# jgsimard/big-dreamer

Measured on AMD Instinct MI355X. Metric: latent transitions/sec (RSSM + imagination) at batch=50 chunk=50 H=15, higher is better.
Workload: dtype f32

## Files before the change

### big_dreamer_amd/_cabi.py

```python
from __future__ import annotations

import ctypes as C
import os

import torch

_HERE = os.path.dirname(os.path.abspath(__file__))
LIB_PATH = os.environ.get("BD_LIB") or os.path.join(_HERE, "libbigdreamer_hip.so")

if not os.path.exists(LIB_PATH):
    raise ImportError(
        f"{LIB_PATH} is missing: the MI355X HIP extension has not been built "
        "(run `python -c 'import __graft_entry__ as g; g.build()'`). There is no CPU fallback.")

lib = C.CDLL(LIB_PATH)

BD_MAX_LAYERS = 6
ACT_NONE, ACT_ELU, ACT_ELU_GRAD = 0, 1, 2
ACT_RELU, ACT_RELU_GRAD, ACT_TANH, ACT_TANH_GRAD = 3, 4, 5, 6
CNN_ACTS = {"ELU": (ACT_ELU, ACT_ELU_GRAD), "ReLU": (ACT_RELU, ACT_RELU_GRAD), "Tanh": (ACT_TANH, ACT_TANH_GRAD)}
GRAD_ACTS = (ACT_ELU_GRAD, ACT_RELU_GRAD, ACT_TANH_GRAD)
P = C.c_void_p
F32 = C.c_float
I32 = C.c_int
# ... 265 lines not shown
    "bd_actor_entropy_rng": (I32, [C.c_ulonglong, C.c_ulonglong, C.c_uint, P, P, I32, I32, I32, I32, P]),
    "bd_gemm_nt": (I32, [P, I32, P, I32, P, I32, I32, I32, I32, I32, P]),
    "bd_categorical_head_forward": (I32, [P, P, I32, I32, I32, P, P, P]),
    "bd_categorical_head_backward": (I32, [P, P, I32, I32, I32, P, P]),
    "bd_kl_categorical_forward": (I32, [P, P, I32, I32, I32, F32, I32, P, I32, P, P]),
    "bd_kl_categorical_backward": (I32, [P, P, I32, I32, I32, F32, F32, F32, F32, P, I32, P, P, P]),
    "bd_plan_rollout": (I32, [C.POINTER(PlanArgs), P]),
    "bd_cem_refit": (I32, [P, I32, P, I32, I32, I32, I32, I32, P, P, P]),
    "bd_plan_rollout_cat": (I32, [C.POINTER(PlanCatArgs), P]),
    "bd_act_step_supported": (I32, [I32, I32, I32, I32, I32, I32]),
    "bd_act_step": (I32, [C.POINTER(ActArgs), P]),
    "bd_act_step_cat_supported": (I32, [I32] * 10),
    "bd_act_step_cat": (I32, [C.POINTER(ActCatArgs), P]),
    "bd_tanh_normal_mode": (I32, [P, P, P, C.c_ulonglong, C.c_ulonglong, C.c_uint, I32, I32, I32, P, P, P]),
    "bd_lambda_return_backward": (I32, [P, F32, I32, I32, F32, F32, P, P, P]),
    "bd_img_heads_supported": (I32, [I32, I32]),
    "bd_img_heads_fwd_bwd": (I32, [C.POINTER(ImgHeadsArgs), P]),
    "bd_actor_reinforce": (I32, [P, P, P, P, P, P, P, I32, I32, I32, F32, F32, F32, I32, P, P, I32, P, P]),
    "bd_actor_reinforce_cat": (I32, [P, P, P, P, P, P, I32, I32, I32, F32, F32, F32, I32, P, P, I32, P, P]),
    "bd_normal_nll": (I32, [P, I32, P, I32, I32, I32, F32, P, I32, P, I32, P, P]),
    "bd_bernoulli_nll": (I32, [P, P, C.c_size_t, F32, P, P, I32, P, P]),
    "bd_kl_forward": (I32, [P, P, P, P, I32, I32, F32, I32, P, I32, P, P]),
    "bd_kl_backward": (I32, [P, P, P, P, I32, I32, F32, F32, F32, F32, P, I32, P, P, P, P, P]),
    "bd_sum": (I32, [P, C.c_size_t, P, I32, P, P]),
    "bd_sumsq": (I32, [P, C.c_size_t, P, I32, P, P]),
    "bd_adam_step": (I32, [P, P, P, P, C.c_size_t, F32, F32, F32, F32, F32, I32, F32, P, I32, P]),
    "bd_polyak": (I32, [P, P, C.c_size_t, F32, P]),
    "bd_replay_gather": (I32, [P, P, I32, I32, P, P]),
    "bd_replay_gather_pixels": (I32, [P, P, I32, I32, I32, P, P, P]),
    "bd_replay_gather_pixels_rng": (I32, [P, P, I32, I32, I32, C.c_ulonglong, C.c_ulonglong, P, P]),
    "bd_replay_append": (I32, [C.POINTER(ReplayAppendArgs), P]),
    "bd_replay_sample_gather": (I32, [C.POINTER(ReplaySampleArgs), P]),
    "bd_reduce_ws_floats": (C.c_size_t, []),
    "bd_conv_gemm": (I32, [C.POINTER(ConvArgs), P]),
    "bd_conv_thin_forward": (I32, [P, I32, I32, I32, I32, I32, P, I32, P, I32, P, P, P]),
    "bd_conv_pack_class": (I32, [P, P, I32, I32, I32, I32, I32, I32, I32, P]),
    "bd_conv_pack_fused": (I32, [P, P, I32, I32, I32, P]),
    "bd_act_backward": (I32, [P, P, C.c_size_t, I32, P]),
    "bd_elu_backward": (I32, [P, P, C.c_size_t, P]),
    "bd_image_layout": (I32, [P, P, I32, I32, I32, I32, P]),
    "bd_eval_frame": (I32, [P, P, I32, U8P, I32, I32, P]),
    "bd_openl_video": (I32, [P, P, I32, I32, U8P, P]),
    "bd_openl_error": (I32, [P, P, I32, I32, I32, I32, P, P]),
    "bd_colsum_ws_floats": (C.c_size_t, [I32]),
    "bd_colsum": (I32, [P, C.c_size_t, I32, P, P, P]),
    "bd_fingerprint": (I32, [C.POINTER(FingerprintArgs), P, P]),
    "bd_diag_ws_floats": (C.c_size_t, []),
    "bd_moments": (I32, [C.POINTER(MomentsArgs), P, P, P]),
    "bd_latent_stats": (I32, [P, P, P, P, I32, I32, P, P, P, P]),
    "bd_latent_stats_categorical": (I32, [P, P, I32, I32, I32, P, P, P, P, P]),
    "bd_segment_sumsq": (I32, [P, I32, C.POINTER(C.c_size_t), P, P, P]),
    "bd_return_range": (I32, [P, I32, I32, I32, C.c_double, C.c_double, P, P, P]),
    "bd_return_seed": (I32, [P, F32, P, C.c_size_t, P, P, I32, P]),
    "bd_actor_reinforce_norm": (I32, [P, P, P, P, P, P, P, P, I32, I32, I32, F32, F32, F32, I32, P, P, I32, P, P]),
    "bd_actor_reinforce_cat_norm": (I32, [P, P, P, P, P, P, P, I32, I32, I32, F32, F32, F32, I32, P, P, I32, P, P]),
    "bd_twohot_decode": (I32, [P, I32, I32, I32, F32, P, P, P]),
    "bd_twohot_decode_backward": (I32, [P, I32, P, I32, I32, F32, P, I32, P]),
    "bd_twohot_nll": (I32, [P, I32, P, P, I32, I32, F32, F32, P, I32, P, P, P]),
}

for _name, (_res, _args) in _SIGS.items():
    _fn = getattr(lib, _name)
    _fn.restype = _res
    _fn.argtypes = _args

EXPORTED = tuple(_SIGS)
# ... 25 lines not shown
```

### big_dreamer_amd/csrc/cabi.hip

```cpp
#include "bd_device.h"
#include "bd_host.h"
#include "bd_rng.h"

namespace bd {
char* err_buf() {
    static thread_local char buf[512] = "";
    return buf;
}

constexpr int kPackThreads = 256, kPackWaves = kPackThreads / 64;
constexpr int kPackCopyX = 16;
constexpr int kPackProdX = 192;
constexpr int kPackE = 256;
struct alignas(16) PackLds {
    float a[16][kPackE + 1];
    float b[kPackE][16];
    float part[kPackWaves][16][17];
};
__device__ __forceinline__ void pack_product(const bd_pack_desc& d, int bx, int nx, PackLds& L) {
    const int Nb = (d.N + 15) >> 4, Kb = (d.K + 15) >> 4;
    const int tid = threadIdx.x, wave = tid >> 6, lane = tid & 63;
    const float* __restrict__ A = d.src;
    const float* __restrict__ B = d.src2;
    const bool vec = ((reinterpret_cast<uintptr_t>(A) | reinterpret_cast<uintptr_t>(B)) & 15) == 0 && (d.ld & 3) == 0 &&
// ... 113 lines not shown
    }
}
template <bool RNG>
__global__ __launch_bounds__(256) void gather_pixels_kernel(const unsigned char* __restrict__ src,
                                                            const int64_t* __restrict__ idx, int n_idx, int pixels,
                                                            float inv_q, float inv_b, const float* __restrict__ noise,
                                                            float* __restrict__ dst, Rng rng) {
    const int quads = pixels >> 2;
    const size_t total = (size_t)n_idx * quads;
    for (size_t e = (size_t)blockIdx.x * blockDim.x + threadIdx.x; e < total; e += (size_t)gridDim.x * blockDim.x) {
        const size_t r = e / quads, q = e - r * quads;
        const uchar4 u = reinterpret_cast<const uchar4*>(src + (size_t)idx[r] * pixels)[q];
        floatx4 nz;
        if constexpr (RNG) {
            const Philox4 p = philox4x32_10((uint32_t)e, (uint32_t)(e >> 32), rng.stream, rng.step, rng.k0, rng.k1);
#pragma unroll
            for (int j = 0; j < 4; ++j) nz[j] = (float)(p.x[j] >> 8) * (1.0f / 16777216.0f);
        } else {
            nz = reinterpret_cast<const floatx4*>(noise)[e];
        }
        floatx4 o;
        o[0] = floorf((float)u.x * inv_q) * inv_b - 0.5f + nz[0] * inv_b;
        o[1] = floorf((float)u.y * inv_q) * inv_b - 0.5f + nz[1] * inv_b;
        o[2] = floorf((float)u.z * inv_q) * inv_b - 0.5f + nz[2] * inv_b;
        o[3] = floorf((float)u.w * inv_q) * inv_b - 0.5f + nz[3] * inv_b;
        reinterpret_cast<floatx4*>(dst)[e] = o;
    }
}
}

extern "C" {

const char* bd_last_error(void) { return bd::err_buf(); }
int bd_version(void) { return 3; }

size_t bd_packed_floats(int N, int K) { return (size_t)bd::cdiv(N, 16) * bd::cdiv(K, 16) * 256; }

int bd_pack_weights(const bd_pack_desc* descs, int n, void* stream) {
    const int n_prod = n > 0 ? n / BD_PACK_PRODUCTS : 0;
    n = n > 0 ? n % BD_PACK_PRODUCTS : n;
    BD_REQUIRE(descs != nullptr && n > 0 && n_prod <= n, "bd_pack_weights: no descriptors");
    hipLaunchKernelGGL(bd::pack_kernel, dim3((n - n_prod) * bd::kPackCopyX + n_prod * bd::kPackProdX), dim3(bd::kPackThreads),
                       n_prod > 0 ? sizeof(bd::PackLds) : 0, (hipStream_t)stream, descs, n - n_prod);
    BD_CHECK_LAUNCH("bd_pack_weights");
    return 0;
}

int bd_replay_gather(const float* src, const int64_t* idx, int n_idx, int width, float* dst, void* stream) {
    BD_REQUIRE(src && idx && dst && n_idx > 0 && width > 0, "bd_replay_gather: bad arguments");
    const size_t total = (size_t)n_idx * width;
    const int blocks = (int)((total + 255) / 256 < 2048 ? (total + 255) / 256 : 2048);
    hipLaunchKernelGGL(bd::gather_rows_kernel, dim3(blocks), dim3(256), 0, (hipStream_t)stream, src, idx, n_idx, width, dst);
    BD_CHECK_LAUNCH("bd_replay_gather");
    return 0;
}

int bd_replay_gather_pixels(const unsigned char* src, const int64_t* idx, int n_idx, int pixels, int bit_depth,
                            const float* noise, float* dst, void* stream) {
    BD_REQUIRE(src && idx && noise && dst && n_idx > 0 && pixels > 0 && (pixels & 3) == 0 && bit_depth >= 1 && bit_depth <= 8,
               "bd_replay_gather_pixels: bad arguments");
    const size_t total = (size_t)n_idx * (pixels >> 2);
    const int blocks = (int)((total + 255) / 256 < 4096 ? (total + 255) / 256 : 4096);
    hipLaunchKernelGGL(bd::gather_pixels_kernel<false>, dim3(blocks), dim3(256), 0, (hipStream_t)stream, src, idx, n_idx, pixels,
                       1.0f / (float)(1 << (8 - bit_depth)), 1.0f / (float)(1 << bit_depth), noise, dst, bd::Rng{0, 0, 0, 0});
    BD_CHECK_LAUNCH("bd_replay_gather_pixels");
    return 0;
}
// ... 16 lines not shown
```

### big_dreamer_amd/csrc/reduce.hip

```cpp
#include "bd_device.h"
#include "bd_host.h"
#include "bd_discrete.h"
#include "bd_latent.h"

namespace bd {

constexpr int kRedBlocks = 1024;
constexpr float kHalfLog2Pi = 0.91893853320467274178f;

static inline int red_blocks(size_t n) {
    size_t b = (n + 255) / 256;
    return (int)(b < 1 ? 1 : (b > kRedBlocks ? kRedBlocks : b));
}

__global__ __launch_bounds__(256) void final_sum_kernel(const double* __restrict__ partials, int n,
                                                        float* __restrict__ scalars, int slot) {
    __shared__ double red[kWaves];
    double s = 0.0;
    for (int i = threadIdx.x; i < n; i += blockDim.x) s += partials[i];
    s = block_sum_d(s, red);
    if (threadIdx.x == 0) scalars[slot] = (float)s;
}

template <int MODE>
__global__ __launch_bounds__(256) void sum_kernel(const float* __restrict__ x, size_t n, double* __restrict__ partials) {
    __shared__ double red[kWaves];
    double s = 0.0;
    for (size_t i = (size_t)blockIdx.x * blockDim.x + threadIdx.x; i < n; i += (size_t)gridDim.x * blockDim.x) {
        const float v = x[i];
        s += MODE ? (double)v * v : (double)v;
    }
    s = block_sum_d(s, red);
    if (threadIdx.x == 0) partials[blockIdx.x] = s;
}

__global__ __launch_bounds__(256) void normal_nll_kernel(const float* __restrict__ pred, int ldp,
                                                         const float* __restrict__ target, int ldt, int rows, int D,
                                                         float grad_scale, float* __restrict__ dpred, int ldd,
                                                         double* __restrict__ partials) {
    __shared__ double red[kWaves];
    double s = 0.0;
    const size_t n = (size_t)rows * D;
    for (size_t i = (size_t)blockIdx.x * blockDim.x + threadIdx.x; i < n; i += (size_t)gridDim.x * blockDim.x) {
        const size_t r = i / D, c = i - r * D;
        const float d = pred[r * ldp + c] - target[r * ldt + c];
        s += (double)(0.5f * d * d + kHalfLog2Pi);
        if (dpred) dpred[r * ldd + c] = d * grad_scale;
    }
    s = block_sum_d(s, red);
    if (threadIdx.x == 0) partials[blockIdx.x] = s;
}

__global__ __launch_bounds__(256) void bernoulli_nll_kernel(const float* __restrict__ logits, const float* __restrict__ target,
                                                            size_t n, float grad_scale, float* __restrict__ dlogits,
                                                            double* __restrict__ partials) {
    __shared__ double red[kWaves];
    double s = 0.0;
    for (size_t i = (size_t)blockIdx.x * blockDim.x + threadIdx.x; i < n; i += (size_t)gridDim.x * blockDim.x) {
        const float x = logits[i], t = target[i];
        s += (double)(fmaxf(x, 0.f) - x * t + log1pf(expf(-fabsf(x))));
        if (dlogits) dlogits[i] = (1.f / (1.f + expf(-x)) - t) * grad_scale;
    }
    s = block_sum_d(s, red);
    if (threadIdx.x == 0) partials[blockIdx.x] = s;
}

__global__ __launch_bounds__(256) void kl_fwd_kernel(const float* __restrict__ qm, const float* __restrict__ qs,
                                                     const float* __restrict__ pm, const float* __restrict__ ps,
                                                     int rows, int S, float free_nats, int sum_form,
                                                     double* __restrict__ partials) {
    __shared__ double red[kWaves];
    double s = 0.0;
    if (!sum_form) {
        const size_t n = (size_t)rows * S;
        for (size_t i = (size_t)blockIdx.x * blockDim.x + threadIdx.x; i < n; i += (size_t)gridDim.x * blockDim.x)
            s += (double)kl_elem(qm[i], qs[i], pm[i], ps[i]);
    } else {
        for (size_t r = (size_t)blockIdx.x * blockDim.x + threadIdx.x; r < (size_t)rows;
             r += (size_t)gridDim.x * blockDim.x) {
            float rs = 0.f;
            for (int c = 0; c < S; ++c) {
                const size_t i = r * S + c;
                rs += kl_elem(qm[i], qs[i], pm[i], ps[i]);
            }
            s += (double)fmaxf(rs, free_nats);
        }
    }
    s = block_sum_d(s, red);
    if (threadIdx.x == 0) partials[blockIdx.x] = s;
}

__device__ __forceinline__ float max_grad(float x, float fn) { return x < fn ? 0.f : (x == fn ? 0.5f : 1.f); }

__global__ __launch_bounds__(256) void kl_bwd_kernel(const float* __restrict__ qm, const float* __restrict__ qs,
                                                     const float* __restrict__ pm, const float* __restrict__ ps,
                                                     int rows, int S, float free_nats, float kl_balance, float weight,
                                                     float inv_count, const float* __restrict__ scalars, int slot,
                                                     float* __restrict__ dqm, float* __restrict__ dqs,
                                                     float* __restrict__ dpm, float* __restrict__ dps) {
    const size_t n = (size_t)rows * S;
    const bool sum_form = kl_balance == -1.f;
    float fq, fp;
    if (!sum_form) {
        const float f = max_grad(scalars[slot] * inv_count, free_nats) * weight * inv_count;
        fp = kl_balance * f;
        fq = (1.f - kl_balance) * f;
    } else {
        fq = fp = weight / (float)rows;
    }
    for (size_t i = (size_t)blockIdx.x * blockDim.x + threadIdx.x; i < n; i += (size_t)gridDim.x * blockDim.x) {
        float gq = fq, gp = fp;
        if (sum_form) {
            const size_t r = i / S;
            float rs = 0.f;
            for (int c = 0; c < S; ++c) {
                const size_t j = r * S + c;
                rs += kl_elem(qm[j], qs[j], pm[j], ps[j]);
            }
            const float f = max_grad(rs, free_nats);
            gq *= f;
            gp *= f;
        }
// ... 45 lines not shown
        for (int t = Hm - 1; t >= 0; --t) {
            const float next = (t == Hm - 1) ? boot : value[(size_t)(t + 1) * N + n];
            const float inp = reward[(size_t)t * N + n] + disc * next * one_minus;
            last = inp + dl * last;
            ret[(size_t)t * N + n] = last;
        }
    }
}

__global__ __launch_bounds__(256) void lambda_bwd_kernel(const float* __restrict__ dret, float dconst, int Hm, int N,
                                                         float disc, float lam, float* __restrict__ dreward,
                                                         float* __restrict__ dvalue) {
    const float c = disc * lam, w = disc * (1.f - lam);
    for (int n = blockIdx.x * blockDim.x + threadIdx.x; n < N; n += gridDim.x * blockDim.x) {
        float G = 0.f;
        for (int t = 0; t < Hm; ++t) {
            G = (dret ? dret[(size_t)t * N + n] : dconst) + c * G;
            dreward[(size_t)t * N + n] = G;
            if (t == 0 && Hm > 1) dvalue[n] = 0.f;
            if (t < Hm - 1) {
                dvalue[(size_t)(t + 1) * N + n] = G * w;
            } else {
                const float prev = (Hm > 1) ? dvalue[(size_t)t * N + n] : 0.f;
                dvalue[(size_t)t * N + n] = prev + G * w + c * G;
            }
        }
    }
}

__global__ __launch_bounds__(256) void actor_reinforce_kernel(
    const float* __restrict__ eps, const float* __restrict__ us, const float* __restrict__ stats,
    const float* __restrict__ ret, const float* __restrict__ base0, const float* __restrict__ value,
    const float* __restrict__ weight, const float* __restrict__ ret_scale, int rows, int N, int A, float scale,
    float dentropy, int write, float* __restrict__ dout, double* __restrict__ partials) {
    __shared__ double red[kWaves];
    constexpr float kLn2 = 0.69314718055994531f;
    if (ret_scale) scale /= ret_scale[0];
    double s = 0.0;
    for (int i = blockIdx.x * blockDim.x + threadIdx.x; i < rows; i += gridDim.x * blockDim.x) {
        const float w = weight ? weight[i] : 1.f;
        const float adv = ret[i] - (i < N ? base0[i] : value[i - N]);
        const float c = scale * w * adv;
        const float dent = dentropy * w;
        const float* e = eps + (size_t)i * A;
        const float* uu = us + (size_t)i * 2 * A;
        const float* st = stats + (size_t)i * 4 * A;
        float* d = dout + (size_t)i * 2 * A;
        float l = 0.f;
        for (int j = 0; j < A; ++j) {
            const float ej = e[j], u = uu[j], sd = uu[A + j];
            const float th = st[j], sg = st[A + j];
            const float x = -2.f * u;
            const float sp = fmaxf(x, 0.f) + log1pf(expf(-fabsf(x)));
            l += -0.5f * ej * ej - logf(sd) - kHalfLog2Pi - 2.f * (kLn2 - u - sp);
            const float inv = 1.f / sd, dth = 1.f - th * th;
            float gm = c * (ej * inv) * dth;
            float gr = c * ((ej * ej - 1.f) * inv) * sg;
            if (write) {
                gm += (dent * st[2 * A + j]) * dth;
                gr += (dent * st[3 * A + j]) * sg;
            } else {
                gm += d[j];
                gr += d[A + j];
            }
            d[j] = gm;
            d[A + j] = gr;
        }
        s += (double)(w * l * adv);
    }
    s = block_sum_d(s, red);
    if (threadIdx.x == 0) partials[blockIdx.x] = s;
}

__global__ __launch_bounds__(256) void actor_reinforce_cat_kernel(
    const float* __restrict__ action, const float* __restrict__ stats, const float* __restrict__ ret,
    const float* __restrict__ base0, const float* __restrict__ value, const float* __restrict__ weight,
    const float* __restrict__ ret_scale, int rows, int N, int A, float scale, float dentropy, int write,
    float* __restrict__ dout, double* __restrict__ partials) {
    __shared__ double red[kWaves];
    const int lane = threadIdx.x & 63;
    if (ret_scale) scale /= ret_scale[0];
    const int nw = gridDim.x * (blockDim.x >> 6);
    const bool valid = lane < A;
    double s = 0.0;
    for (int i = blockIdx.x * (blockDim.x >> 6) + (threadIdx.x >> 6); i < rows; i += nw) {
        const float w = weight ? weight[i] : 1.f;
        const float adv = ret[i] - (i < N ? base0[i] : value[i - N]);
        const float c = scale * w * adv;
        const size_t j = (size_t)i * A + lane;
        const float norm = valid ? stats[j] : -INFINITY;
        const unsigned long long hot = __ballot(valid && action[j] > 0.5f);
        const int k = hot ? __builtin_ctzll(hot) : 0;
        const float p = disc_probs(norm, valid);
        const float l = __shfl(norm, k, 64);
        float g = c * ((lane == k ? 1.f : 0.f) - p);
        if (write) {
            const float H = disc_entropy(norm, p, valid);
            g += (dentropy * w) * (-p * (norm + H));
        } else if (valid) {
            g += dout[j];
        }
        if (valid) dout[j] = g;
        if (lane == 0) s += (double)(w * l * adv);
    }
    s = block_sum_d(s, red);
    if (threadIdx.x == 0) partials[blockIdx.x] = s;
}

__global__ __launch_bounds__(256) void adam_kernel(float* __restrict__ p, float* __restrict__ g, float* __restrict__ m,
                                                   float* __restrict__ v, size_t n, float beta1, float beta2, float eps,
                                                   float wd, float step_size, float inv_sqrt_bc2, float max_norm,
                                                   const float* __restrict__ scalars, int sqnorm_slot) {
    const float total_norm = sqrtf(scalars[sqnorm_slot]);
    const float q = max_norm / (total_norm + 1e-6f);
    const float coef = q > 1.f ? 1.f : q;
    for (size_t i = (size_t)blockIdx.x * blockDim.x + threadIdx.x; i < n; i += (size_t)gridDim.x * blockDim.x) {
        const float gc = g[i] * coef;
        g[i] = gc;
        const float pi = p[i];
        const float gw = gc + wd * pi;
        const float mi = m[i] + (1.f - beta1) * (gw - m[i]);
        const float vi = v[i] * beta2 + (1.f - beta2) * gw * gw;
        m[i] = mi;
        v[i] = vi;
        const float denom = sqrtf(vi) * inv_sqrt_bc2 + eps;
        p[i] = pi - step_size * (mi / denom);
    }
}

__global__ __launch_bounds__(256) void polyak_kernel(float* __restrict__ t, const float* __restrict__ s, size_t n, float w) {
    for (size_t i = (size_t)blockIdx.x * blockDim.x + threadIdx.x; i < n; i += (size_t)gridDim.x * blockDim.x)
        t[i] = s[i] * w + t[i] * (1.f - w);
}

__global__ __launch_bounds__(256) void cat_head_fwd_kernel(const float* __restrict__ logits, const float* __restrict__ q,
                                                           size_t groups, int C, float* __restrict__ state,
                                                           float* __restrict__ probs) {
    const int l = threadIdx.x & 31;
    for (size_t g = (size_t)blockIdx.x * 8 + (threadIdx.x >> 5); g < groups; g += (size_t)gridDim.x * 8) {
// ... 29 lines not shown
            if (ob > best || (ob == best && oa < arg)) { best = ob; arg = oa; }
        }
#pragma unroll
        for (int i = 0; i < kCatPer; ++i) {
            const int c = l + 32 * i;
            if (c < C) state[base + c] = (c == arg) ? 1.f : 0.f;
        }
    }
}

__global__ __launch_bounds__(256) void cat_head_bwd_kernel(const float* __restrict__ dstate, const float* __restrict__ probs,
                                                           size_t groups, int C, float* __restrict__ dlogits) {
    const int l = threadIdx.x & 31;
    for (size_t g = (size_t)blockIdx.x * 8 + (threadIdx.x >> 5); g < groups; g += (size_t)gridDim.x * 8) {
        const size_t base = g * C;
        float pr[kCatPer], gr[kCatPer], dot = 0.f;
#pragma unroll
        for (int i = 0; i < kCatPer; ++i) {
            const int c = l + 32 * i;
            pr[i] = c < C ? probs[base + c] : 0.f;
            gr[i] = c < C ? dstate[base + c] : 0.f;
            dot += pr[i] * gr[i];
        }
        dot = half_sum(dot);
#pragma unroll
        for (int i = 0; i < kCatPer; ++i) {
            const int c = l + 32 * i;
            if (c < C) dlogits[base + c] = pr[i] * (gr[i] - dot);
        }
    }
}

__global__ __launch_bounds__(256) void cat_kl_fwd_kernel(const float* __restrict__ ql, const float* __restrict__ pl, int rows,
                                                         int D, int C, float free_nats, int sum_form,
                                                         double* __restrict__ partials) {
    __shared__ double red[kWaves > 4 ? kWaves : 4];
    const int l = threadIdx.x & 31;
    const size_t units = sum_form ? (size_t)rows : (size_t)rows * D;
    const int per = sum_form ? D : 1;
    double acc = 0.0;
    for (size_t u = (size_t)blockIdx.x * 8 + (threadIdx.x >> 5); u < units; u += (size_t)gridDim.x * 8) {
        float rs = 0.f;
        for (int d = 0; d < per; ++d) {
            const size_t base = (u * per + d) * C;
            float lq[kCatPer], lp[kCatPer];
            group_log_softmax(ql + base, C, l, lq);
            group_log_softmax(pl + base, C, l, lp);
            rs += group_kl(lq, lp, C, l);
        }
        if (l == 0) acc += (double)(sum_form ? fmaxf(rs, free_nats) : rs);
    }
    acc = block_sum_d(acc, red);
    if (threadIdx.x == 0) partials[blockIdx.x] = acc;
}

__global__ __launch_bounds__(256) void cat_kl_bwd_kernel(const float* __restrict__ ql, const float* __restrict__ pl, int rows,
                                                         int D, int C, float free_nats, float kl_balance, float weight,
                                                         float inv_count, const float* __restrict__ scalars, int slot,
                                                         float* __restrict__ dql, float* __restrict__ dpl) {
    const int l = threadIdx.x & 31;
    const bool sum_form = kl_balance == -1.f;
    const size_t units = sum_form ? (size_t)rows : (size_t)rows * D;
    const int per = sum_form ? D : 1;
    float fq, fp;
    if (!sum_form) {
        const float f = max_grad(scalars[slot] * inv_count, free_nats) * weight * inv_count;
        fp = kl_balance * f;
        fq = (1.f - kl_balance) * f;
    } else {
        fq = fp = weight / (float)rows;
    }
    for (size_t u = (size_t)blockIdx.x * 8 + (threadIdx.x >> 5); u < units; u += (size_t)gridDim.x * 8) {
        float f = 1.f;
        if (sum_form) {
            float rs = 0.f;
            for (int d = 0; d < per; ++d) {
                const size_t base = (u * per + d) * C;
                float lq[kCatPer], lp[kCatPer];
                group_log_softmax(ql + base, C, l, lq);
                group_log_softmax(pl + base, C, l, lp);
                rs += group_kl(lq, lp, C, l);
            }
            f = max_grad(rs, free_nats);
        }
        for (int d = 0; d < per; ++d) {
            const size_t base = (u * per + d) * C;
            float lq[kCatPer], lp[kCatPer];
            group_log_softmax(ql + base, C, l, lq);
            group_log_softmax(pl + base, C, l, lp);
            const float kl = group_kl(lq, lp, C, l);
#pragma unroll
            for (int i = 0; i < kCatPer; ++i) {
                const int c = l + 32 * i;
                if (c < C) {
                    const float qv = expf(lq[i]), pv = expf(lp[i]);
                    dql[base + c] = f * fq * (qv == 0.f ? 0.f : qv * (lq[i] - lp[i] - kl));
                    dpl[base + c] = f * fp * (pv - qv);
                }
            }
        }
    }
}

static int finish(double* partials, int nb, float* scalars, int slot, hipStream_t s, const char* name) {
    hipLaunchKernelGGL(final_sum_kernel, dim3(1), dim3(256), 0, s, partials, nb, scalars, slot);
    BD_CHECK_LAUNCH(name);
    return 0;
}

}

extern "C" {
using namespace bd;

size_t bd_reduce_ws_floats(void) { return 2 * (size_t)kRedBlocks; }

int bd_sum(const float* x, size_t n, float* scalars, int slot, float* ws, void* stream) {
    BD_REQUIRE(x && scalars && ws && n > 0, "bd_sum: bad arguments");
    const int nb = red_blocks(n);
    hipLaunchKernelGGL(sum_kernel<0>, dim3(nb), dim3(256), 0, (hipStream_t)stream, x, n, (double*)ws);
    BD_CHECK_LAUNCH("bd_sum");
    return finish((double*)ws, nb, scalars, slot, (hipStream_t)stream, "bd_sum(final)");
}

int bd_actor_reinforce_norm(const float* eps_action, const float* act_us, const float* act_stats, const float* returns,
                            const float* base0, const float* value, const float* weight, const float* ret_scale, int Hm,
                            int N, int A, float rho, float grad_scale, float dentropy, int write, float* d_actor_out,
                            float* scalars, int slot, float* ws, void* stream) {
    BD_REQUIRE(eps_action && act_us && act_stats && returns && base0 && (value || Hm == 1) && d_actor_out && scalars && ws,
               "bd_actor_reinforce: missing pointers");
    BD_REQUIRE(Hm > 0 && N > 0 && A > 0 && (size_t)Hm * N <= (size_t)INT32_MAX / 4 && slot >= 0,
               "bd_actor_reinforce: bad dims (Hm=%d N=%d A=%d slot=%d)", Hm, N, A, slot);
    BD_REQUIRE(rho >= 0.f && rho <= 1.f, "bd_actor_reinforce: gradient mixing %g outside [0, 1]", (double)rho);
    BD_REQUIRE(((size_t)ret_scale & 3u) == 0, "bd_actor_reinforce: ret_scale is not 4-byte aligned");
    const int rows = Hm * N;
    const int nb = red_blocks((size_t)rows);
    hipLaunchKernelGGL(actor_reinforce_kernel, dim3(nb), dim3(256), 0, (hipStream_t)stream, eps_action, act_us, act_stats,
                       returns, base0, value, weight, ret_scale, rows, N, A, -(1.f - rho) * grad_scale, dentropy, write,
                       d_actor_out, (double*)ws);
    BD_CHECK_LAUNCH("bd_actor_reinforce");
    return finish((double*)ws, nb, scalars, slot, (hipStream_t)stream, "bd_actor_reinforce(final)");
}

int bd_actor_reinforce(const float* eps_action, const float* act_us, const float* act_stats, const float* returns,
                       const float* base0, const float* value, const float* weight, int Hm, int N, int A, float rho,
                       float grad_scale, float dentropy, int write, float* d_actor_out, float* scalars, int slot, float* ws,
                       void* stream) {
    return bd_actor_reinforce_norm(eps_action, act_us, act_stats, returns, base0, value, weight, nullptr, Hm, N, A, rho,
                                   grad_scale, dentropy, write, d_actor_out, scalars, slot, ws, stream);
}

int bd_actor_reinforce_cat_norm(const float* action, const float* act_stats, const float* returns, const float* base0,
                                const float* value, const float* weight, const float* ret_scale, int Hm, int N, int A,
                                float rho, float grad_scale, float dentropy, int write, float* d_actor_out, float* scalars,
                                int slot, float* ws, void* stream) {
    BD_REQUIRE(action && act_stats && returns && base0 && (value || Hm == 1) && d_actor_out && scalars && ws,
               "bd_actor_reinforce_cat: missing pointers");
    BD_REQUIRE(Hm > 0 && N > 0 && A > 0 && A <= 64 && (size_t)Hm * N <= (size_t)INT32_MAX / 4 && slot >= 0,
               "bd_actor_reinforce_cat: bad dims (Hm=%d N=%d A=%d slot=%d)", Hm, N, A, slot);
    BD_REQUIRE(rho >= 0.f && rho <= 1.f, "bd_actor_reinforce_cat: gradient mixing %g outside [0, 1]", (double)rho);
    BD_REQUIRE(((size_t)ret_scale & 3u) == 0, "bd_actor_reinforce_cat: ret_scale is not 4-byte aligned");
    const int rows = Hm * N;
    const int nb = red_blocks((size_t)rows);
    hipLaunchKernelGGL(actor_reinforce_cat_kernel, dim3(nb), dim3(256), 0, (hipStream_t)stream, action, act_stats, returns,
                       base0, value, weight, ret_scale, rows, N, A, -(1.f - rho) * grad_scale, dentropy, write, d_actor_out,
                       (double*)ws);
    BD_CHECK_LAUNCH("bd_actor_reinforce_cat");
    return finish((double*)ws, nb, scalars, slot, (hipStream_t)stream, "bd_actor_reinforce_cat(final)");
}

int bd_actor_reinforce_cat(const float* action, const float* act_stats, const float* returns, const float* base0,
                           const float* value, const float* weight, int Hm, int N, int A, float rho, float grad_scale,
                           float dentropy, int write, float* d_actor_out, float* scalars, int slot, float* ws,
                           void* stream) {
    return bd_actor_reinforce_cat_norm(action, act_stats, returns, base0, value, weight, nullptr, Hm, N, A, rho, grad_scale,
                                       dentropy, write, d_actor_out, scalars, slot, ws, stream);
}

int bd_sumsq(const float* x, size_t n, float* scalars, int slot, float* ws, void* stream) {
    BD_REQUIRE(x && scalars && ws && n > 0, "bd_sumsq: bad arguments");
    const int nb = red_blocks(n);
    hipLaunchKernelGGL(sum_kernel<1>, dim3(nb), dim3(256), 0, (hipStream_t)stream, x, n, (double*)ws);
    BD_CHECK_LAUNCH("bd_sumsq");
    return finish((double*)ws, nb, scalars, slot, (hipStream_t)stream, "bd_sumsq(final)");
}

int bd_normal_nll(const float* pred, int ldp, const float* target, int ldt, int rows, int D, float grad_scale,
                  float* dpred, int ldd, float* scalars, int slot, float* ws, void* stream) {
    BD_REQUIRE(pred && target && scalars && ws && rows > 0 && D > 0, "bd_normal_nll: bad arguments");
    BD_REQUIRE(ldp >= D && ldt >= D && (!dpred || ldd >= D), "bd_normal_nll: leading dimension too small");
    const int nb = red_blocks((size_t)rows * D);
    hipLaunchKernelGGL(normal_nll_kernel, dim3(nb), dim3(256), 0, (hipStream_t)stream, pred, ldp, target, ldt, rows, D,
                       grad_scale, dpred, ldd, (double*)ws);
    BD_CHECK_LAUNCH("bd_normal_nll");
    return finish((double*)ws, nb, scalars, slot, (hipStream_t)stream, "bd_normal_nll(final)");
}

int bd_bernoulli_nll(const float* logits, const float* target, size_t n, float grad_scale, float* dlogits, float* scalars,
                     int slot, float* ws, void* stream) {
    BD_REQUIRE(logits && target && scalars && ws && n > 0, "bd_bernoulli_nll: bad arguments");
    const int nb = red_blocks(n);
    hipLaunchKernelGGL(bernoulli_nll_kernel, dim3(nb), dim3(256), 0, (hipStream_t)stream, logits, target, n, grad_scale,
                       dlogits, (double*)ws);
    BD_CHECK_LAUNCH("bd_bernoulli_nll");
    return finish((double*)ws, nb, scalars, slot, (hipStream_t)stream, "bd_bernoulli_nll(final)");
}

int bd_kl_forward(const float* qm, const float* qs, const float* pm, const float* ps, int rows, int S, float free_nats,
                  int sum_form, float* scalars, int slot, float* ws, void* stream) {
    BD_REQUIRE(qm && qs && pm && ps && scalars && ws && rows > 0 && S > 0, "bd_kl_forward: bad arguments");
    const int nb = red_blocks(sum_form ? (size_t)rows : (size_t)rows * S);
    hipLaunchKernelGGL(kl_fwd_kernel, dim3(nb), dim3(256), 0, (hipStream_t)stream, qm, qs, pm, ps, rows, S, free_nats,
                       sum_form, (double*)ws);
    BD_CHECK_LAUNCH("bd_kl_forward");
    return finish((double*)ws, nb, scalars, slot, (hipStream_t)stream, "bd_kl_forward(final)");
}

int bd_kl_backward(const float* qm, const float* qs, const float* pm, const float* ps, int rows, int S, float free_nats,
                   float kl_balance, float weight, float inv_count, const float* scalars, int slot, float* dqm,
                   float* dqs, float* dpm, float* dps, void* stream) {
    BD_REQUIRE(qm && qs && pm && ps && scalars && dqm && dqs && dpm && dps && rows > 0 && S > 0,
               "bd_kl_backward: bad arguments");
    hipLaunchKernelGGL(kl_bwd_kernel, dim3(red_blocks((size_t)rows * S)), dim3(256), 0, (hipStream_t)stream, qm, qs, pm,
                       ps, rows, S, free_nats, kl_balance, weight, inv_count, scalars, slot, dqm, dqs, dpm, dps);
    BD_CHECK_LAUNCH("bd_kl_backward");
    return 0;
}

int bd_gauss_head_forward(const float* out, const float* eps, int M, int S, float min_std, float* mean, float* std,
                          float* state, void* stream) {
    BD_REQUIRE(out && M > 0 && S > 0 && (!state || eps), "bd_gauss_head_forward: bad arguments");
    hipLaunchKernelGGL(gauss_head_fwd_kernel, dim3(red_blocks((size_t)M * S)), dim3(256), 0, (hipStream_t)stream, out, eps,
                       M, S, min_std, mean, std, state);
    BD_CHECK_LAUNCH("bd_gauss_head_forward");
    return 0;
}

int bd_gauss_head_backward(const float* out, const float* eps, const float* dstate, const float* dmean,
                           const float* dstd, int M, int S, float* dout, void* stream) {
    BD_REQUIRE(out && dout && M > 0 && S > 0 && (!dstate || eps), "bd_gauss_head_backward: bad arguments");
    hipLaunchKernelGGL(gauss_head_bwd_kernel, dim3(red_blocks((size_t)M * S)), dim3(256), 0, (hipStream_t)stream, out, eps,
                       dstate, dmean, dstd, M, S, dout);
    BD_CHECK_LAUNCH("bd_gauss_head_backward");
    return 0;
}

int bd_lambda_return_forward(const float* reward, const float* value, int Hm, int N, float discount, float lambda_,
                             float* returns, void* stream) {
// ... 32 lines not shown

static inline int cat_blocks(size_t units) {
    size_t b = (units + 7) / 8;
    return (int)(b < 1 ? 1 : (b > (size_t)kRedBlocks ? (size_t)kRedBlocks : b));
}

int bd_categorical_head_forward(const float* logits, const float* q_noise, int rows, int D, int C, float* state,
                                float* probs, void* stream) {
    BD_REQUIRE(logits && q_noise && state && probs && rows > 0 && D > 0, "bd_categorical_head_forward: bad arguments");
    BD_REQUIRE(C > 0 && C <= 32 * kCatPer, "bd_categorical_head_forward: %d classes (max %d)", C, 32 * kCatPer);
    const size_t groups = (size_t)rows * D;
    hipLaunchKernelGGL(cat_head_fwd_kernel, dim3(cat_blocks(groups)), dim3(256), 0, (hipStream_t)stream, logits, q_noise,
                       groups, C, state, probs);
    BD_CHECK_LAUNCH("bd_categorical_head_forward");
    return 0;
}

int bd_categorical_head_backward(const float* dstate, const float* probs, int rows, int D, int C, float* dlogits,
                                 void* stream) {
    BD_REQUIRE(dstate && probs && dlogits && rows > 0 && D > 0, "bd_categorical_head_backward: bad arguments");
    BD_REQUIRE(C > 0 && C <= 32 * kCatPer, "bd_categorical_head_backward: %d classes (max %d)", C, 32 * kCatPer);
    const size_t groups = (size_t)rows * D;
    hipLaunchKernelGGL(cat_head_bwd_kernel, dim3(cat_blocks(groups)), dim3(256), 0, (hipStream_t)stream, dstate, probs,
                       groups, C, dlogits);
    BD_CHECK_LAUNCH("bd_categorical_head_backward");
    return 0;
}

int bd_kl_categorical_forward(const float* post_logits, const float* prior_logits, int rows, int D, int C, float free_nats,
                              int sum_form, float* scalars, int slot, float* ws, void* stream) {
    BD_REQUIRE(post_logits && prior_logits && scalars && ws && rows > 0 && D > 0, "bd_kl_categorical_forward: bad arguments");
    BD_REQUIRE(C > 0 && C <= 32 * kCatPer, "bd_kl_categorical_forward: %d classes (max %d)", C, 32 * kCatPer);
    const int nb = cat_blocks(sum_form ? (size_t)rows : (size_t)rows * D);
    hipLaunchKernelGGL(cat_kl_fwd_kernel, dim3(nb), dim3(256), 0, (hipStream_t)stream, post_logits, prior_logits, rows, D, C,
                       free_nats, sum_form, (double*)ws);
    BD_CHECK_LAUNCH("bd_kl_categorical_forward");
    return finish((double*)ws, nb, scalars, slot, (hipStream_t)stream, "bd_kl_categorical_forward(final)");
}

int bd_kl_categorical_backward(const float* post_logits, const float* prior_logits, int rows, int D, int C, float free_nats,
                               float kl_balance, float weight, float inv_count, const float* scalars, int slot,
                               float* dpost, float* dprior, void* stream) {
    BD_REQUIRE(post_logits && prior_logits && scalars && dpost && dprior && rows > 0 && D > 0,
               "bd_kl_categorical_backward: bad arguments");
    BD_REQUIRE(C > 0 && C <= 32 * kCatPer, "bd_kl_categorical_backward: %d classes (max %d)", C, 32 * kCatPer);
    const bool sum_form = kl_balance == -1.f;
    hipLaunchKernelGGL(cat_kl_bwd_kernel, dim3(cat_blocks(sum_form ? (size_t)rows : (size_t)rows * D)), dim3(256), 0,
                       (hipStream_t)stream, post_logits, prior_logits, rows, D, C, free_nats, kl_balance, weight, inv_count,
                       scalars, slot, dpost, dprior);
    BD_CHECK_LAUNCH("bd_kl_categorical_backward");
    return 0;
}

}
```

### include/bigdreamer_hip.h

```cpp
#ifndef BIGDREAMER_HIP_H
#define BIGDREAMER_HIP_H

#include <stddef.h>
#include <stdint.h>

#ifdef __cplusplus
extern "C" {
#endif

#define BD_MAX_LAYERS 6
#define BD_ACT_NONE 0
#define BD_ACT_ELU 1
#define BD_ACT_ELU_GRAD 2
#define BD_ACT_RELU 3
#define BD_ACT_RELU_GRAD 4
#define BD_ACT_TANH 5
#define BD_ACT_TANH_GRAD 6

const char* bd_last_error(void);
int bd_version(void);

#define BD_PACK_COPY 0
#define BD_PACK_PRODUCT 1
#define BD_PACK_PRODUCT_VEC 2
// ... 541 lines not shown
    float* dst_reward;
    float* dst_nonterminal;
} bd_replay_append_args;
int bd_replay_append(const bd_replay_append_args* a, void* stream);

typedef struct {
    const void* obs;
    const float* act;
    const float* reward;
    const float* nonterminal;
    int obs_width;
    int A;
    int size;
    int lanes;
    int lane_size;
    int idx;
    int full;
    int n;
    int L;
    int bit_depth;
    unsigned long long seed;
    unsigned long long step;
    unsigned long long pix_seed;
    unsigned long long pix_step;
    float* dst_obs;
    float* dst_act;
    float* dst_reward;
    float* dst_nonterminal;
    int64_t* idx_out;
} bd_replay_sample_args;
int bd_replay_sample_gather(const bd_replay_sample_args* a, void* stream);

size_t bd_reduce_ws_floats(void);

#define BD_FP_MAX_BUFFERS 16
typedef struct {
    int n_buf;
    struct {
        const float* p;
        size_t n;
    } buf[BD_FP_MAX_BUFFERS];
} bd_fingerprint_args;
int bd_fingerprint(const bd_fingerprint_args* a, unsigned long long* out, void* stream);

size_t bd_diag_ws_floats(void);

#define BD_MOMENTS_MAX_BUFFERS 16
#define BD_MOMENTS_WORDS 6
typedef struct {
    int n_buf;
    struct {
        const float* p;
        const float* q;
        size_t n;
    } buf[BD_MOMENTS_MAX_BUFFERS];
} bd_moments_args;
int bd_moments(const bd_moments_args* a, double* out, float* ws, void* stream);

#define BD_LATENT_WORDS 15
int bd_latent_stats(const float* qm, const float* qs, const float* pm, const float* ps, int rows, int S, double* out,
                    double* colsum, float* ws, void* stream);

#define BD_LATENT_CAT_WORDS 5
int bd_latent_stats_categorical(const float* post_logits, const float* prior_logits, int rows, int D, int C, double* out,
                                double* colsum, unsigned* used, float* ws, void* stream);

// ... 19 lines not shown
```

Baseline: 13.92 million.

## Fuse reduction finalisation into one launch with a last-block ticket

Reduction kernels (sum, sumsq, NLL, KL, actor reinforce) now finish the reduction themselves. Each block writes its partial, fences, and takes an atomic ticket; the last block to arrive sums all partials and writes the scalar. This removes the separate single-block final_sum launch whenever the grid has at most 320 blocks, cutting per-loss launch overhead and a serial dependency. In exchange it adds atomics and fences and relies on the self-wrapping ticket counter starting at zero; a mode switch and a reset entry point allow falling back to the two-launch path.

```diff
diff --git a/big_dreamer_amd/_cabi.py b/big_dreamer_amd/_cabi.py
--- a/big_dreamer_amd/_cabi.py
+++ b/big_dreamer_amd/_cabi.py
@@ -321,6 +321,8 @@
     "bd_replay_append": (I32, [C.POINTER(ReplayAppendArgs), P]),
     "bd_replay_sample_gather": (I32, [C.POINTER(ReplaySampleArgs), P]),
     "bd_reduce_ws_floats": (C.c_size_t, []),
+    "bd_reduce_set_two_launch": (I32, [I32]),
+    "bd_reduce_reset": (I32, [C.c_void_p, C.c_void_p]),
     "bd_conv_gemm": (I32, [C.POINTER(ConvArgs), P]),
     "bd_conv_thin_forward": (I32, [P, I32, I32, I32, I32, I32, P, I32, P, I32, P, P, P]),
     "bd_conv_pack_class": (I32, [P, P, I32, I32, I32, I32, I32, I32, I32, P]),
diff --git a/big_dreamer_amd/csrc/cabi.hip b/big_dreamer_amd/csrc/cabi.hip
--- a/big_dreamer_amd/csrc/cabi.hip
+++ b/big_dreamer_amd/csrc/cabi.hip
@@ -169,7 +169,7 @@
 extern "C" {
 
 const char* bd_last_error(void) { return bd::err_buf(); }
-int bd_version(void) { return 3; }
+int bd_version(void) { return 4; }
 
 size_t bd_packed_floats(int N, int K) { return (size_t)bd::cdiv(N, 16) * bd::cdiv(K, 16) * 256; }
 
diff --git a/big_dreamer_amd/csrc/reduce.hip b/big_dreamer_amd/csrc/reduce.hip
--- a/big_dreamer_amd/csrc/reduce.hip
+++ b/big_dreamer_amd/csrc/reduce.hip
@@ -6,6 +6,9 @@
 namespace bd {
 
 constexpr int kRedBlocks = 1024;
+#ifndef BD_RED_TICKET_MAX
+#define BD_RED_TICKET_MAX 320
+#endif
 constexpr float kHalfLog2Pi = 0.91893853320467274178f;
 
 static inline int red_blocks(size_t n) {
@@ -13,63 +16,111 @@
     return (int)(b < 1 ? 1 : (b > kRedBlocks ? kRedBlocks : b));
 }
 
-__global__ __launch_bounds__(256) void final_sum_kernel(const double* __restrict__ partials, int n,
-                                                        float* __restrict__ scalars, int slot) {
-    __shared__ double red[kWaves];
+constexpr int kRedFinal = 1;
+constexpr int kRedWarm = 2;
+constexpr int kRedTicketMax = BD_RED_TICKET_MAX;
+constexpr int kTicketFloat = 2 * kRedBlocks;
+constexpr int kTicketFloats = 4;
+
+struct RedOut {
+    double* partials;
+    unsigned* ticket;
+    float* scalars;
+    int slot;
+    int flags;
+};
+
+__device__ __forceinline__ void final_sum(const double* partials, int n, float* scalars, int slot, double* red) {
     double s = 0.0;
     for (int i = threadIdx.x; i < n; i += blockDim.x) s += partials[i];
     s = block_sum_d(s, red);
     if (threadIdx.x == 0) scalars[slot] = (float)s;
 }
 
+__global__ __launch_bounds__(256) void final_sum_kernel(const double* __restrict__ partials, int n,
+                                                        float* __restrict__ scalars, int slot) {
+    __shared__ double red[kWaves];
+    final_sum(partials, n, scalars, slot, red);
+}
+
+__device__ __forceinline__ void reduce_finish(const RedOut& o, double s) {
+    __shared__ double red[kWaves > 4 ? kWaves : 4];
+    __shared__ unsigned last;
+    const unsigned nb = gridDim.x;
+    if (o.flags & kRedWarm) {
+        double w = 0.0;
+        for (unsigned i = threadIdx.x; i < nb; i += blockDim.x) w += o.partials[i];
+        asm volatile("" ::"v"(w));
+    }
+    s = block_sum_d(s, red);
+    if (!(o.flags & kRedFinal)) {
+        if (threadIdx.x == 0) o.partials[blockIdx.x] = s;
+        return;
+    }
+    if (nb == 1) {
+        if (threadIdx.x == 0) {
+            o.partials[0] = s;
+            o.scalars[o.slot] = (float)(0.0 + s);
+        }
+        return;
+    }
+    if (threadIdx.x == 0) {
+        o.partials[blockIdx.x] = s;
+        asm volatile("s_waitcnt vmcnt(0)" ::: "memory");
+        __builtin_amdgcn_fence(__ATOMIC_RELEASE, "agent");
+        asm volatile("s_waitcnt vmcnt(0)" ::: "memory");
+        const unsigned top = nb - 1;
+        unsigned t = atomicInc(o.ticket, top);
+        if (t > top) t = atomicInc(o.ticket, top);
+        if (t == top) {
+            __builtin_amdgcn_fence(__ATOMIC_ACQUIRE, "agent");
+            asm volatile("s_waitcnt vmcnt(0)" ::: "memory");
+        }
+        last = t == top;
+    }
+    __syncthreads();
+    if (last) final_sum(o.partials, (int)nb, o.scalars, o.slot, red);
+}
+
 template <int MODE>
-__global__ __launch_bounds__(256) void sum_kernel(const float* __restrict__ x, size_t n, double* __restrict__ partials) {
-    __shared__ double red[kWaves];
+__global__ __launch_bounds__(256) void sum_kernel(const float* __restrict__ x, size_t n, RedOut o) {
     double s = 0.0;
     for (size_t i = (size_t)blockIdx.x * blockDim.x + threadIdx.x; i < n; i += (size_t)gridDim.x * blockDim.x) {
         const float v = x[i];
         s += MODE ? (double)v * v : (double)v;
     }
-    s = block_sum_d(s, red);
-    if (threadIdx.x == 0) partials[blockIdx.x] = s;
+    reduce_finish(o, s);
 }
 
 __global__ __launch_bounds__(256) void normal_nll_kernel(const float* __restrict__ pred, int ldp,
                                                          const float* __restrict__ target, int ldt, int rows, int D,
-                                                         float grad_scale, float* __restrict__ dpred, int ldd,
-                                                         double* __restrict__ partials) {
-    __shared__ double red[kWaves];
+                                                         float grad_scale, float* __restrict__ dpred, int ldd, RedOut o) {
+    const size_t n = (size_t)rows * D;
     double s = 0.0;
-    const size_t n = (size_t)rows * D;
     for (size_t i = (size_t)blockIdx.x * blockDim.x + threadIdx.x; i < n; i += (size_t)gridDim.x * blockDim.x) {
         const size_t r = i / D, c = i - r * D;
         const float d = pred[r * ldp + c] - target[r * ldt + c];
         s += (double)(0.5f * d * d + kHalfLog2Pi);
         if (dpred) dpred[r * ldd + c] = d * grad_scale;
     }
-    s = block_sum_d(s, red);
-    if (threadIdx.x == 0) partials[blockIdx.x] = s;
+    reduce_finish(o, s);
 }
 
 __global__ __launch_bounds__(256) void bernoulli_nll_kernel(const float* __restrict__ logits, const float* __restrict__ target,
                                                             size_t n, float grad_scale, float* __restrict__ dlogits,
-                                                            double* __restrict__ partials) {
-    __shared__ double red[kWaves];
+                                                            RedOut o) {
     double s = 0.0;
     for (size_t i = (size_t)blockIdx.x * blockDim.x + threadIdx.x; i < n; i += (size_t)gridDim.x * blockDim.x) {
         const float x = logits[i], t = target[i];
         s += (double)(fmaxf(x, 0.f) - x * t + log1pf(expf(-fabsf(x))));
         if (dlogits) dlogits[i] = (1.f / (1.f + expf(-x)) - t) * grad_scale;
     }
-    s = block_sum_d(s, red);
-    if (threadIdx.x == 0) partials[blockIdx.x] = s;
+    reduce_finish(o, s);
 }
 
 __global__ __launch_bounds__(256) void kl_fwd_kernel(const float* __restrict__ qm, const float* __restrict__ qs,
                                                      const float* __restrict__ pm, const float* __restrict__ ps,
-                                                     int rows, int S, float free_nats, int sum_form,
-                                                     double* __restrict__ partials) {
-    __shared__ double red[kWaves];
+                                                     int rows, int S, float free_nats, int sum_form, RedOut o) {
     double s = 0.0;
     if (!sum_form) {
         const size_t n = (size_t)rows * S;
@@ -86,8 +137,7 @@
             s += (double)fmaxf(rs, free_nats);
         }
     }
-    s = block_sum_d(s, red);
-    if (threadIdx.x == 0) partials[blockIdx.x] = s;
+    reduce_finish(o, s);
 }
 
 __device__ __forceinline__ float max_grad(float x, float fn) { return x < fn ? 0.f : (x == fn ? 0.5f : 1.f); }
@@ -199,8 +249,7 @@
     const float* __restrict__ eps, const float* __restrict__ us, const float* __restrict__ stats,
     const float* __restrict__ ret, const float* __restrict__ base0, const float* __restrict__ value,
     const float* __restrict__ weight, const float* __restrict__ ret_scale, int rows, int N, int A, float scale,
-    float dentropy, int write, float* __restrict__ dout, double* __restrict__ partials) {
-    __shared__ double red[kWaves];
+    float dentropy, int write, float* __restrict__ dout, RedOut o) {
     constexpr float kLn2 = 0.69314718055994531f;
     if (ret_scale) scale /= ret_scale[0];
     double s = 0.0;
@@ -235,16 +284,14 @@
         }
         s += (double)(w * l * adv);
     }
-    s = block_sum_d(s, red);
-    if (threadIdx.x == 0) partials[blockIdx.x] = s;
+    reduce_finish(o, s);
 }
 
 __global__ __launch_bounds__(256) void actor_reinforce_cat_kernel(
     const float* __restrict__ action, const float* __restrict__ stats, const float* __restrict__ ret,
     const float* __restrict__ base0, const float* __restrict__ value, const float* __restrict__ weight,
     const float* __restrict__ ret_scale, int rows, int N, int A, float scale, float dentropy, int write,
-    float* __restrict__ dout, double* __restrict__ partials) {
-    __shared__ double red[kWaves];
+    float* __restrict__ dout, RedOut o) {
     const int lane = threadIdx.x & 63;
     if (ret_scale) scale /= ret_scale[0];
     const int nw = gridDim.x * (blockDim.x >> 6);
@@ -270,8 +317,7 @@
         if (valid) dout[j] = g;
         if (lane == 0) s += (double)(w * l * adv);
     }
-    s = block_sum_d(s, red);
-    if (threadIdx.x == 0) partials[blockIdx.x] = s;
+    reduce_finish(o, s);
 }
 
 __global__ __launch_bounds__(256) void adam_kernel(float* __restrict__ p, float* __restrict__ g, float* __restrict__ m,
@@ -367,9 +413,7 @@
 }
 
 __global__ __launch_bounds__(256) void cat_kl_fwd_kernel(const float* __restrict__ ql, const float* __restrict__ pl, int rows,
-                                                         int D, int C, float free_nats, int sum_form,
-                                                         double* __restrict__ partials) {
-    __shared__ double red[kWaves > 4 ? kWaves : 4];
+                                                         int D, int C, float free_nats, int sum_form, RedOut o) {
     const int l = threadIdx.x & 31;
     const size_t units = sum_form ? (size_t)rows : (size_t)rows * D;
     const int per = sum_form ? D : 1;
@@ -385,8 +429,7 @@
         }
         if (l == 0) acc += (double)(sum_form ? fmaxf(rs, free_nats) : rs);
     }
-    acc = block_sum_d(acc, red);
-    if (threadIdx.x == 0) partials[blockIdx.x] = acc;
+    reduce_finish(o, acc);
 }
 
 __global__ __launch_bounds__(256) void cat_kl_bwd_kernel(const float* __restrict__ ql, const float* __restrict__ pl, int rows,
@@ -437,8 +480,17 @@
     }
 }
 
-static int finish(double* partials, int nb, float* scalars, int slot, hipStream_t s, const char* name) {
-    hipLaunchKernelGGL(final_sum_kernel, dim3(1), dim3(256), 0, s, partials, nb, scalars, slot);
+static int red_mode = 0;
+
+static RedOut red_out(int nb, float* scalars, int slot, float* ws) {
+    const bool one = red_mode != 1 && nb <= kRedTicketMax;
+    return RedOut{(double*)ws, (unsigned*)(ws + kTicketFloat), scalars, slot,
+                  one ? (kRedFinal | (red_mode == 2 ? kRedWarm : 0)) : 0};
+}
+
+static int finish(const RedOut& o, int nb, hipStream_t s, const char* name) {
+    if (o.flags & kRedFinal) return 0;
+    hipLaunchKernelGGL(final_sum_kernel, dim3(1), dim3(256), 0, s, o.partials, nb, o.scalars, o.slot);
     BD_CHECK_LAUNCH(name);
     return 0;
 }
@@ -448,14 +500,28 @@
 extern "C" {
 using namespace bd;
 
-size_t bd_reduce_ws_floats(void) { return 2 * (size_t)kRedBlocks; }
+size_t bd_reduce_ws_floats(void) { return (size_t)kTicketFloat + kTicketFloats; }
+
+int bd_reduce_set_two_launch(int mode) {
+    BD_REQUIRE(mode >= 0 && mode <= 2, "bd_reduce_set_two_launch: mode %d", mode);
+    bd::red_mode = mode;
+    return 0;
+}
+
+int bd_reduce_reset(float* ws, void* stream) {
+    BD_REQUIRE(ws, "bd_reduce_reset: no workspace");
+    BD_REQUIRE(hipMemsetAsync(ws + kTicketFloat, 0, kTicketFloats * sizeof(float), (hipStream_t)stream) == hipSuccess,
+               "bd_reduce_reset: memset failed");
+    return 0;
+}
 
 int bd_sum(const float* x, size_t n, float* scalars, int slot, float* ws, void* stream) {
     BD_REQUIRE(x && scalars && ws && n > 0, "bd_sum: bad arguments");
     const int nb = red_blocks(n);
-    hipLaunchKernelGGL(sum_kernel<0>, dim3(nb), dim3(256), 0, (hipStream_t)stream, x, n, (double*)ws);
+    const RedOut o = red_out(nb, scalars, slot, ws);
+    hipLaunchKernelGGL(sum_kernel<0>, dim3(nb), dim3(256), 0, (hipStream_t)stream, x, n, o);
     BD_CHECK_LAUNCH("bd_sum");
-    return finish((double*)ws, nb, scalars, slot, (hipStream_t)stream, "bd_sum(final)");
+    return finish(o, nb, (hipStream_t)stream, "bd_sum(final)");
 }
 
 int bd_actor_reinforce_norm(const float* eps_action, const float* act_us, const float* act_stats, const float* returns,
@@ -470,11 +536,12 @@
     BD_REQUIRE(((size_t)ret_scale & 3u) == 0, "bd_actor_reinforce: ret_scale is not 4-byte aligned");
     const int rows = Hm * N;
     const int nb = red_blocks((size_t)rows);
+    const RedOut o = red_out(nb, scalars, slot, ws);
     hipLaunchKernelGGL(actor_reinforce_kernel, dim3(nb), dim3(256), 0, (hipStream_t)stream, eps_action, act_us, act_stats,
                        returns, base0, value, weight, ret_scale, rows, N, A, -(1.f - rho) * grad_scale, dentropy, write,
-                       d_actor_out, (double*)ws);
+                       d_actor_out, o);
     BD_CHECK_LAUNCH("bd_actor_reinforce");
-    return finish((double*)ws, nb, scalars, slot, (hipStream_t)stream, "bd_actor_reinforce(final)");
+    return finish(o, nb, (hipStream_t)stream, "bd_actor_reinforce(final)");
 }
 
 int bd_actor_reinforce(const float* eps_action, const float* act_us, const float* act_stats, const float* returns,
@@ -497,11 +564,12 @@
     BD_REQUIRE(((size_t)ret_scale & 3u) == 0, "bd_actor_reinforce_cat: ret_scale is not 4-byte aligned");
     const int rows = Hm * N;
     const int nb = red_blocks((size_t)rows);
+    const RedOut o = red_out(nb, scalars, slot, ws);
     hipLaunchKernelGGL(actor_reinforce_cat_kernel, dim3(nb), dim3(256), 0, (hipStream_t)stream, action, act_stats, returns,
                        base0, value, weight, ret_scale, rows, N, A, -(1.f - rho) * grad_scale, dentropy, write, d_actor_out,
-                       (double*)ws);
+                       o);
     BD_CHECK_LAUNCH("bd_actor_reinforce_cat");
-    return finish((double*)ws, nb, scalars, slot, (hipStream_t)stream, "bd_actor_reinforce_cat(final)");
+    return finish(o, nb, (hipStream_t)stream, "bd_actor_reinforce_cat(final)");
 }
 
 int bd_actor_reinforce_cat(const float* action, const float* act_stats, const float* returns, const float* base0,
@@ -515,9 +583,10 @@
 int bd_sumsq(const float* x, size_t n, float* scalars, int slot, float* ws, void* stream) {
     BD_REQUIRE(x && scalars && ws && n > 0, "bd_sumsq: bad arguments");
     const int nb = red_blocks(n);
-    hipLaunchKernelGGL(sum_kernel<1>, dim3(nb), dim3(256), 0, (hipStream_t)stream, x, n, (double*)ws);
+    const RedOut o = red_out(nb, scalars, slot, ws);
+    hipLaunchKernelGGL(sum_kernel<1>, dim3(nb), dim3(256), 0, (hipStream_t)stream, x, n, o);
     BD_CHECK_LAUNCH("bd_sumsq");
-    return finish((double*)ws, nb, scalars, slot, (hipStream_t)stream, "bd_sumsq(final)");
+    return finish(o, nb, (hipStream_t)stream, "bd_sumsq(final)");
 }
 
 int bd_normal_nll(const float* pred, int ldp, const float* target, int ldt, int rows, int D, float grad_scale,
@@ -525,30 +594,33 @@
     BD_REQUIRE(pred && target && scalars && ws && rows > 0 && D > 0, "bd_normal_nll: bad arguments");
     BD_REQUIRE(ldp >= D && ldt >= D && (!dpred || ldd >= D), "bd_normal_nll: leading dimension too small");
     const int nb = red_blocks((size_t)rows * D);
+    const RedOut o = red_out(nb, scalars, slot, ws);
     hipLaunchKernelGGL(normal_nll_kernel, dim3(nb), dim3(256), 0, (hipStream_t)stream, pred, ldp, target, ldt, rows, D,
-                       grad_scale, dpred, ldd, (double*)ws);
+                       grad_scale, dpred, ldd, o);
     BD_CHECK_LAUNCH("bd_normal_nll");
-    return finish((double*)ws, nb, scalars, slot, (hipStream_t)stream, "bd_normal_nll(final)");
+    return finish(o, nb, (hipStream_t)stream, "bd_normal_nll(final)");
 }
 
 int bd_bernoulli_nll(const float* logits, const float* target, size_t n, float grad_scale, float* dlogits, float* scalars,
                      int slot, float* ws, void* stream) {
     BD_REQUIRE(logits && target && scalars && ws && n > 0, "bd_bernoulli_nll: bad arguments");
     const int nb = red_blocks(n);
+    const RedOut o = red_out(nb, scalars, slot, ws);
     hipLaunchKernelGGL(bernoulli_nll_kernel, dim3(nb), dim3(256), 0, (hipStream_t)stream, logits, target, n, grad_scale,
-                       dlogits, (double*)ws);
+                       dlogits, o);
     BD_CHECK_LAUNCH("bd_bernoulli_nll");
-    return finish((double*)ws, nb, scalars, slot, (hipStream_t)stream, "bd_bernoulli_nll(final)");
+    return finish(o, nb, (hipStream_t)stream, "bd_bernoulli_nll(final)");
 }
 
 int bd_kl_forward(const float* qm, const float* qs, const float* pm, const float* ps, int rows, int S, float free_nats,
                   int sum_form, float* scalars, int slot, float* ws, void* stream) {
     BD_REQUIRE(qm && qs && pm && ps && scalars && ws && rows > 0 && S > 0, "bd_kl_forward: bad arguments");
     const int nb = red_blocks(sum_form ? (size_t)rows : (size_t)rows * S);
+    const RedOut o = red_out(nb, scalars, slot, ws);
     hipLaunchKernelGGL(kl_fwd_kernel, dim3(nb), dim3(256), 0, (hipStream_t)stream, qm, qs, pm, ps, rows, S, free_nats,
-                       sum_form, (double*)ws);
+                       sum_form, o);
     BD_CHECK_LAUNCH("bd_kl_forward");
-    return finish((double*)ws, nb, scalars, slot, (hipStream_t)stream, "bd_kl_forward(final)");
+    return finish(o, nb, (hipStream_t)stream, "bd_kl_forward(final)");
 }
 
 int bd_kl_backward(const float* qm, const float* qs, const float* pm, const float* ps, int rows, int S, float free_nats,
@@ -647,10 +719,11 @@
     BD_REQUIRE(post_logits && prior_logits && scalars && ws && rows > 0 && D > 0, "bd_kl_categorical_forward: bad arguments");
     BD_REQUIRE(C > 0 && C <= 32 * kCatPer, "bd_kl_categorical_forward: %d classes (max %d)", C, 32 * kCatPer);
     const int nb = cat_blocks(sum_form ? (size_t)rows : (size_t)rows * D);
+    const RedOut o = red_out(nb, scalars, slot, ws);
     hipLaunchKernelGGL(cat_kl_fwd_kernel, dim3(nb), dim3(256), 0, (hipStream_t)stream, post_logits, prior_logits, rows, D, C,
-                       free_nats, sum_form, (double*)ws);
+                       free_nats, sum_form, o);
     BD_CHECK_LAUNCH("bd_kl_categorical_forward");
-    return finish((double*)ws, nb, scalars, slot, (hipStream_t)stream, "bd_kl_categorical_forward(final)");
+    return finish(o, nb, (hipStream_t)stream, "bd_kl_categorical_forward(final)");
 }
 
 int bd_kl_categorical_backward(const float* post_logits, const float* prior_logits, int rows, int D, int C, float free_nats,
diff --git a/include/bigdreamer_hip.h b/include/bigdreamer_hip.h
--- a/include/bigdreamer_hip.h
+++ b/include/bigdreamer_hip.h
@@ -597,6 +597,8 @@
 int bd_replay_sample_gather(const bd_replay_sample_args* a, void* stream);
 
 size_t bd_reduce_ws_floats(void);
+int bd_reduce_reset(float* ws, void* stream);
+int bd_reduce_set_two_launch(int mode);
 
 #define BD_FP_MAX_BUFFERS 16
 typedef struct {
```

Result: no change. 13.90 million (-0.1%).
